# goldbricklemon/uplift-upsample-3dhpe

Hardware: AMD Instinct MI355X
Metric: pose-sequences/sec (higher is better)
Workload: dtype f16x3 (f32 operands split into f16 hi/lo, 3 MFMA passes, f32 accumulate); 1 GPU; config/h36m_351.json forward, N=71 tokens (receptive field 351), J=17, batch 128/GPU, s_in=5, seeded Keras-default weights; global_batch=128, parallelism=batch-sharded x1, hipgraph=True, concurrent_half_batches=False, batches_in_flight=8

## Files before the change

### uplift-upsample-3dhpe_amd/build.py

```python
import os
import subprocess
import sys

HERE = os.path.dirname(os.path.abspath(__file__))
CSRC = os.path.join(HERE, "csrc")
LIB = os.path.join(CSRC, "libuu3d.so")
SOURCES = ["uu3d_api.hip", "uu3d_ops.hip"]
HEADERS = ["uu3d_tchain16.h", "uu3d_gemm.h", "uu3d_gemm_h3.h", "uu3d_gemm_panel.h", "uu3d_gemm_panel8.h", "uu3d_gemm_wt.h", "uu3d_mlp_fused.h", "uu3d_attn.h", "uu3d_attn_h3.h", "uu3d_attn_long.h", "uu3d_spatial.h", "uu3d_spatial_h3.h", "uu3d_pk.h", "uu3d_misc.h", "uu3d_train.h", "uu3d_bwd.h", "uu3d_launch.h", "uu3d_train_kernels.h", "uu3d_dropout.h", "uu3d_train_step.inc", os.path.join("..", "..", "include", "uu3d_ops.h"), os.path.join("..", "..", "include", "uu3d.h")]


def _fingerprint(extra_flags=()):
    import hashlib
    h = hashlib.sha256()
    for f in SOURCES + HEADERS:
        h.update(f.encode()); h.update(open(os.path.join(CSRC, f), "rb").read())
    h.update(repr((DEVICE_FLAGS, tuple(extra_flags))).encode())
    try:
        h.update(subprocess.run([os.environ.get("HIPCC", "/opt/rocm/bin/hipcc"), "--version"], capture_output=True, text=True).stdout.encode())
    except OSError:
        pass
    return h.hexdigest()


def _stale(lib, extra_flags=()):
    stamp = lib + ".sha256"
    if not os.path.exists(lib) or not os.path.exists(stamp):
        return True
    return open(stamp).read().strip() != _fingerprint(extra_flags)


DEVICE_FLAGS = ["-Xclang", "-target-feature", "-Xclang", "-packed-fp32-ops"]
_HOST_NOISE = "is not a recognized feature for this target"


TIMING_LIB = os.path.join(CSRC, "libuu3d_timing.so")


def build(force=False, verbose=False, extra_flags=(), timing=False):
    lib = TIMING_LIB if timing else LIB
    extra_flags = tuple(extra_flags) + (("-DUU3D_TIMING_BUILD",) if timing else ())
    if not force and not _stale(lib, extra_flags):
        return lib
    hipcc = os.environ.get("HIPCC", "/opt/rocm/bin/hipcc")
    cmd = [hipcc, "-O3", "-std=c++17", "--offload-arch=gfx950", "-shared", "-fPIC",
           "-Wall", "-Wno-unused-function", *DEVICE_FLAGS, *extra_flags,
           "-o", lib] + [os.path.join(CSRC, s) for s in SOURCES]
    if verbose:
        print(" ".join(cmd), flush=True)
    r = subprocess.run(cmd, cwd=CSRC, stderr=subprocess.PIPE, text=True)
    err = "".join(l for l in r.stderr.splitlines(True) if _HOST_NOISE not in l)
    if err.strip():
        sys.stderr.write(err)
    if r.returncode != 0:
        raise subprocess.CalledProcessError(r.returncode, cmd)
    with open(lib + ".sha256", "w") as f:
        f.write(_fingerprint(extra_flags) + "\n")
    return lib


if __name__ == "__main__":
    print(build(force="--force" in sys.argv, verbose=True, timing="--timing" in sys.argv))
# ... 1 lines not shown
```

### uplift-upsample-3dhpe_amd/csrc/uu3d_api.hip

```cpp
#include <hip/hip_runtime.h>

#include <algorithm>
#include <cmath>
#include <cstdio>
#include <cstdlib>
#include <cstring>
#include <functional>
#include <map>
#include <string>
#include <vector>

#include "../../include/uu3d.h"
#include "uu3d_gemm.h"
#include "uu3d_gemm_h3.h"
#include "uu3d_gemm_panel.h"
#include <mutex>
#include "uu3d_gemm_panel8.h"
#include "uu3d_gemm_wt.h"
#include "uu3d_mlp_fused.h"
#include "uu3d_tchain16.h"
#include "uu3d_attn.h"
#include "uu3d_attn_h3.h"
#include "uu3d_spatial.h"
#include "uu3d_spatial_h3.h"
#include "uu3d_misc.h"
#include "uu3d_train.h"
#include "uu3d_bwd.h"
#include "uu3d_launch.h"
#include "uu3d_train_kernels.h"

using namespace uu3d;

namespace {

constexpr int kJ = 17, kDS = 32, kHS = 64, kHeads = 8, kDH = 48;
using SLY = SpatialBlockLayout<kDS, kHS>;
using SLY2 = SpatialBlockLayoutV2<kDS, kHS>;
constexpr int kFR = 3;
#ifndef UU3D_SPATIAL_MT
#define UU3D_SPATIAL_MT 1
#endif
constexpr int kSpatialMT = UU3D_SPATIAL_MT;

std::string g_create_error;

inline int round_up(int v, int m) { return (v + m - 1) / m * m; }
inline size_t align_up(size_t v, size_t a) { return (v + a - 1) / a * a; }

struct WeightRec {
    std::string name;
    std::vector<int64_t> dims;
    int64_t numel = 0;
    std::vector<float> host;
    bool set = false;
};

struct BlockDev {
    const float *ln1_g, *ln1_b, *wqkv_t, *bqkv, *wp_t, *bp, *ln2_g, *ln2_b, *w1_t, *b1, *w2_t, *b2;
    const float* pe;
    size_t wqkv_pf = 0, w1_pf = 0;
    size_t w2_mf = 0;
    size_t wp_pf = 0;
};

struct ProfRec {
    std::string name, kernel;
    double flops, bytes;
    hipEvent_t e0, e1;
};

}

struct uu3d_train_state;
struct uu3d_model {
    uu3d_config cfg;
    uu3d_train_state* ts = nullptr;
    int device = 0;
    std::vector<WeightRec> weights;
    std::map<std::string, int> index;
    std::vector<int> L;
    bool committed = false;
    bool generic = false;
    float* gparams = nullptr;
    float* arena = nullptr;
    size_t arena_floats = 0;
    bool no_mlpf = false;
    bool no_wt = false;
    bool attn_f32 = false;
    bool attn_wg = false;
    bool no_panel = false;
    bool no_panel_proj = false;
    bool throughput = false;
    struct TcLaunch { int flags; size_t w_off ; size_t p_off ; };
    std::vector<TcLaunch> tchain;
    int tchain_mode = -1;
    int tchain_min_tiles = 8;
    bool tchain_short = true;
    int num_cus = 256;
    std::recursive_mutex train_mu;
    bool in_commit = false;
    int* d_range = nullptr;
    bool no_planes = false;
    _Float16* harena = nullptr;
    size_t harena_halfs = 0;
    std::map<size_t, std::pair<size_t, size_t>> hplanes;
    std::map<size_t, size_t> panel_off, mlpf_off;
    SpatialParams sp{};
    const float* sp_blocks_v1 = nullptr;
    const float* sp_blocks_v2 = nullptr;
    bool spatial_valu = false;
    bool spatial_f32 = false;
    bool spatial_h3_always = false;
    size_t sp_frag_off = 0;
    const float *s2t_wt = nullptr, *s2t_b = nullptr, *token = nullptr, *pe_t = nullptr;
    std::vector<BlockDev> tblocks, sblocks;
    const float *h1_wt = nullptr, *h1_b = nullptr, *h2_wt = nullptr, *h2_b = nullptr;
    bool profiling = false;
    std::vector<ProfRec> prof;
    size_t prof_used = 0;
    std::string err;
};

namespace {

inline bool tchain_possible(const uu3d_config& c) {
    return c.precision == UU3D_PREC_F16X3 && c.d_temporal == 384 && c.h_temporal == 768 && c.num_heads == 8 && c.temporal_depth >= 1;
}

int fail(uu3d_model* m, int code, const std::string& msg) {
    if (m) m->err = msg; else g_create_error = msg;
    return code;
}

#define HIPCHK(m, expr)                                                                         \
    do {                                                                                        \
        hipError_t e__ = (expr);                                                                \
        if (e__ != hipSuccess)                                                                  \
            return fail(m, UU3D_ERR_HIP, std::string(#expr) + ": " + hipGetErrorString(e__));   \
    } while (0)

void add_weight(uu3d_model* m, const std::string& name, std::vector<int64_t> dims) {
    WeightRec r;
    r.name = name;
    r.dims = dims;
    r.numel = 1;
    for (auto d : dims) r.numel *= d;
    m->index[name] = (int)m->weights.size();
    m->weights.push_back(std::move(r));
}

void add_block(uu3d_model* m, const std::string& p, int d, int h, bool strided, bool qkv_bias) {
    add_weight(m, p + "/norm1/gamma", {d});
    add_weight(m, p + "/norm1/beta", {d});
    for (const char* nm : {"wq", "wk", "wv"}) {
        add_weight(m, p + "/attn/" + nm + "/kernel", {d, d});
        if (qkv_bias) add_weight(m, p + "/attn/" + nm + "/bias", {d});
    }
    add_weight(m, p + "/attn/projection/kernel", {d, d});
    add_weight(m, p + "/attn/projection/bias", {d});
    add_weight(m, p + "/norm2/gamma", {d});
    add_weight(m, p + "/norm2/beta", {d});
    if (strided) {
        add_weight(m, p + "/mlp/fc1/kernel", {1, d, h});
        add_weight(m, p + "/mlp/fc1/bias", {h});
        add_weight(m, p + "/mlp/strided_conv/kernel", {3, h, d});
        add_weight(m, p + "/mlp/strided_conv/bias", {d});
// ... 105 lines not shown
    if (generic) {
        if (c->num_heads < 1 || c->d_spatial < 1 || c->d_temporal < 1 || c->h_spatial < 1 || c->h_temporal < 1)
            return fail(nullptr, UU3D_ERR_INVALID_ARGUMENT, "dims and head count must be positive");
        if (c->d_spatial % c->num_heads != 0 || c->d_temporal % c->num_heads != 0)
            return fail(nullptr, UU3D_ERR_INVALID_ARGUMENT, "embed dims must be divisible by NUM_HEADS (vision_transformer.py:79)");
        if (!attn_generic_head_dim_ok(c->d_spatial / c->num_heads) || !attn_generic_head_dim_ok(c->d_temporal / c->num_heads))
            return fail(nullptr, UU3D_ERR_UNSUPPORTED, "generic forward: head dims (embed dim / NUM_HEADS) must be one of 2, 4, 8, 12, 16, 24, 32, 48, 64");
        if (c->d_spatial % 4 != 0 || c->d_temporal % 4 != 0 || c->h_spatial % 4 != 0)
            return fail(nullptr, UU3D_ERR_UNSUPPORTED, "generic forward: embed dims and MLP widths must be multiples of 4 (16-byte row pieces in every loader)");
        if (c->num_keypoints > 128 || c->num_frames > 128)
            return fail(nullptr, UU3D_ERR_UNSUPPORTED, "generic forward: at most 128 keypoints and 128 frames");
        if (c->temporal_depth < 1 || c->num_strided < 1 || !c->full_output)
            return fail(nullptr, UU3D_ERR_UNSUPPORTED, "generic forward: needs at least one temporal block, one strided block and the full-sequence head");
    }
    if (c->h_temporal % 4 != 0 || c->h_temporal < 4)
        return fail(nullptr, UU3D_ERR_UNSUPPORTED, "h_temporal must be a positive multiple of 4");
    if (c->temporal_depth == 0 && c->has_strided_input && c->num_strided > 0 && c->first_strided_token_attention_layer > 1)
        return fail(nullptr, UU3D_ERR_INVALID_ARGUMENT, "temporal_depth == 0 with FIRST_STRIDED_TOKEN_ATTENTION_LAYER > 1: the reference's key mask has N entries, strided block 2 has fewer keys");
    if (c->d_temporal > 64 * 4 * 4)
        return fail(nullptr, UU3D_ERR_UNSUPPORTED, "d_temporal > 1024");

    int ndev = 0;
    if (hipGetDeviceCount(&ndev) != hipSuccess || device < 0 || device >= ndev)
        return fail(nullptr, UU3D_ERR_NO_DEVICE, "HIP device not available");

    auto* m = new uu3d_model();
    m->cfg = *c;
    m->device = device;
    m->generic = generic;
    m->L.push_back(c->num_frames);
    for (int i = 0; i < c->num_strided; ++i) {
        if (c->strides[i] < 1 || c->pad_left[i] < 0 || c->pad_right[i] < 0) {
            delete m;
            return fail(nullptr, UU3D_ERR_INVALID_ARGUMENT, "bad stride/padding");
        }
        const int Lin = m->L.back();
        const int Lout = (Lin + c->pad_left[i] + c->pad_right[i] - 3) / c->strides[i] + 1;
        if (Lin + c->pad_left[i] + c->pad_right[i] < 3 || Lout < 1) {
            delete m;
            return fail(nullptr, UU3D_ERR_INVALID_ARGUMENT, "strided block reduces the sequence below one token");
        }
        if (Lin > (c->precision == UU3D_PREC_F16X3 ? ATTN_H3_MAX_L : 128)) {
            delete m;
            return fail(nullptr, UU3D_ERR_UNSUPPORTED, c->precision == UU3D_PREC_F16X3 ? "sequence length > 416 tokens" : "sequence length > 128 tokens with precision f32");
        }
        m->L.push_back(Lout);
    }
    if (c->num_strided > 0 && m->L.back() != 1) {
        delete m;
        return fail(nullptr, UU3D_ERR_INVALID_ARGUMENT, "STRIDES/PADDINGS must reduce the sequence to one token");
    }
    build_inventory(m);
    { const char* e = getenv("UU3D_SPATIAL"); m->spatial_valu = (e != nullptr && std::string(e) == "valu");
      m->spatial_f32 = (e != nullptr && std::string(e) == "f32"); m->spatial_h3_always = (e != nullptr && std::string(e) == "h3"); }
    { const char* e = getenv("UU3D_NO_PLANES"); m->no_planes = (e != nullptr && e[0] == '1'); }
    { const char* e = getenv("UU3D_ATTN_WG"); m->attn_wg = (e != nullptr && e[0] == '1'); }
    { const char* e = getenv("UU3D_NO_MLPF"); m->no_mlpf = (e != nullptr && e[0] == '1'); }
    { const char* e = getenv("UU3D_NO_WT"); m->no_wt = (e != nullptr && e[0] == '1'); }
    { const char* e = getenv("UU3D_ATTN_F32"); m->attn_f32 = (e != nullptr && e[0] == '1'); }
    { const char* e = getenv("UU3D_NO_PANEL"); m->no_panel = (e != nullptr && e[0] == '1'); }
    { const char* e = getenv("UU3D_NO_PANEL_PROJ"); m->no_panel_proj = (e != nullptr && e[0] == '1'); }
    { const char* e = getenv("UU3D_TCHAIN"); if (e != nullptr && (e[0] == '0' || e[0] == '1')) m->tchain_mode = e[0] - '0'; }
    { const char* e = getenv("UU3D_TCHAIN_MIN_TILES"); if (e != nullptr && atoi(e) > 0) m->tchain_min_tiles = atoi(e); }
    { const char* e = getenv("UU3D_TCHAIN_SHORT"); if (e != nullptr) m->tchain_short = atoi(e) != 0; }
    { hipDeviceProp_t pr; if (hipGetDeviceProperties(&pr, device) == hipSuccess && pr.multiProcessorCount > 0) m->num_cus = pr.multiProcessorCount; }
    if (hipSetDevice(device) != hipSuccess) {
        delete m;
        return fail(nullptr, UU3D_ERR_HIP, "hipSetDevice failed");
    }
    if (hipMalloc((void**)&m->d_range, 2 * sizeof(int)) != hipSuccess || hipMemset(m->d_range, 0, 2 * sizeof(int)) != hipSuccess) {
        delete m;
        return fail(nullptr, UU3D_ERR_HIP, "hipMalloc of the range-guard word failed");
    }
    *out = m;
    return UU3D_OK;
}

static void train_free(uu3d_model* m);
static int generic_forward(uu3d_model* m, const float* kp2d, const uint8_t* mask, int32_t B, float* full_out, float* central_out,
                           float* const* attn_out, void* workspace, size_t workspace_bytes, void* stream);
void uu3d_destroy(uu3d_model* m) {
    if (!m) return;
    (void)hipSetDevice(m->device);
    train_free(m);
    if (m->gparams) (void)hipFree(m->gparams);
    if (m->arena) (void)hipFree(m->arena);
    if (m->harena) (void)hipFree(m->harena);
    if (m->d_range) (void)hipFree(m->d_range);
    for (auto& r : m->prof) { (void)hipEventDestroy(r.e0); (void)hipEventDestroy(r.e1); }
    delete m;
}

int uu3d_num_weights(const uu3d_model* m) { return m ? (int)m->weights.size() : 0; }

int uu3d_weight_info(const uu3d_model* m, int i, const char** name, int32_t* ndim, int64_t dims[4]) {
    if (!m || i < 0 || i >= (int)m->weights.size()) return UU3D_ERR_INVALID_ARGUMENT;
    const WeightRec& r = m->weights[i];
    if (name) *name = r.name.c_str();
    if (ndim) *ndim = (int32_t)r.dims.size();
    if (dims) for (size_t k = 0; k < 4; ++k) dims[k] = k < r.dims.size() ? r.dims[k] : 1;
    return UU3D_OK;
}

int uu3d_set_weight(uu3d_model* m, const char* name, const float* data, int64_t numel) {
    if (!m || !name || !data) return fail(m, UU3D_ERR_INVALID_ARGUMENT, "null argument to uu3d_set_weight");
    auto it = m->index.find(name);
    if (it == m->index.end()) return fail(m, UU3D_ERR_INVALID_ARGUMENT, std::string("unknown weight: ") + name);
// ... 241 lines not shown
            add_proj(tb, block_name(true, 0)); add_fc1(tb, block_name(true, 0));
            tcb.push_back(std::move(tb));
        }
    }

    if (m->arena_floats < P.buf.size()) {
        if (m->arena) HIPCHK(m, hipFree(m->arena));
        m->arena = nullptr;
        HIPCHK(m, hipMalloc((void**)&m->arena, P.buf.size() * sizeof(float)));
        m->arena_floats = P.buf.size();
    }
    HIPCHK(m, hipMemcpyAsync(m->arena, P.buf.data(), P.buf.size() * sizeof(float), hipMemcpyHostToDevice, stream));
    HIPCHK(m, hipStreamSynchronize(stream));
    if (c.precision == UU3D_PREC_F16X3) {
        std::vector<_Float16> hb(64, (_Float16)0.f);
        m->hplanes.clear();
        for (auto& d : P.dense) {
            const size_t hi = align_up(hb.size(), 64); hb.resize(hi + d.second);
            const size_t lo = align_up(hb.size(), 64); hb.resize(lo + d.second);
            for (size_t i = 0; i < d.second; ++i) {
                const float x = P.buf[d.first + i];
                if (!(std::fabs(x) < 65504.0f))
                    return fail(m, UU3D_ERR_RANGE, "a Dense / Conv1D kernel holds a value of magnitude >= 65504 (or a non-finite one): not representable by the f16x3 operand planes; build the model with precision f32");
                const _Float16 h = h3_hi(x);
                hb[hi + i] = h; hb[lo + i] = (_Float16)((x - (float)h) * H3_SCALE);
            }
            m->hplanes[d.first] = {hi, lo};
        }
        {
            using FL = SpatialFragLayoutH3;
            m->sp_frag_off = align_up(hb.size(), 64);
            hb.resize(m->sp_frag_off + (size_t)c.spatial_depth * FL::size);
            for (int i = 0; i < c.spatial_depth; ++i) {
                const std::string p = "spatial_block_" + std::to_string(i + 1);
                _Float16* d = hb.data() + m->sp_frag_off + (size_t)i * FL::size;
                auto frag = [&](int off, const std::string& nm, int K, int Nn) {
                    const float* s = W(m, p + nm);
                    for (int nt = 0; nt < Nn / 32; ++nt)
                        for (int kk = 0; kk < K / 16; ++kk)
                            for (int lane = 0; lane < 64; ++lane)
                                for (int e = 0; e < 8; ++e) {
                                    const float x = s[(size_t)(16 * kk + 8 * (lane >> 5) + e) * Nn + 32 * nt + (lane & 31)];
                                    const _Float16 h = h3_hi(x);
                                    const size_t at = (size_t)off + (((size_t)(nt * (K / 16) + kk) * 2) * 64 + lane) * 8 + e;
                                    d[at] = h;
                                    d[at + 64 * 8] = (_Float16)((x - (float)h) * H3_SCALE);
                                }
                };
                frag(FL::fq, "/attn/wq/kernel", ds, ds); frag(FL::fk, "/attn/wk/kernel", ds, ds);
                frag(FL::fv, "/attn/wv/kernel", ds, ds); frag(FL::fp, "/attn/projection/kernel", ds, ds);
                frag(FL::f1, "/mlp/fc1/kernel", ds, kHS); frag(FL::f2, "/mlp/fc2/kernel", kHS, ds);
            }
        }
        m->panel_off.clear();
        if (dt % 192 == 0 && ht % 32 == 0) {
            auto add_panel = [&](size_t bt_off, int Nn, int K = 0, int Kp = 0) {
                if (K == 0) { K = dt; Kp = Kdt; }
                const auto it = m->hplanes.find(bt_off);
                if (it == m->hplanes.end() || K % 384 != 0) return;
                const size_t at = align_up(hb.size(), 64);
                hb.resize(at + panel_b_halfs(Nn, K));
                panel_pack_operand(hb.data() + it->second.first, hb.data() + it->second.second, Nn, K, Kp, hb.data() + at);
                m->panel_off[bt_off] = at;
            };
            for (auto& o : toff) { add_panel(o.wqkv, 3 * dt); add_panel(o.w1, ht); add_panel(o.wp, dt); }
            m->mlpf_off.clear();
            if (dt == 32 * MLPF_OC && ht == 256 * MLPF_SLICES)
                for (auto& o : toff) {
                    const auto it = m->hplanes.find(o.w2);
                    if (it == m->hplanes.end()) continue;
                    const size_t at = align_up(hb.size(), 64);
                    hb.resize(at + mlpf_w2_halfs());
                    mlpf_pack_w2(hb.data() + it->second.first, hb.data() + it->second.second, Kht, hb.data() + at);
                    m->mlpf_off[o.w2] = at;
                }
            for (auto& o : soff) { add_panel(o.wqkv, 3 * dt); add_panel(o.w1, ht); add_panel(o.wp, dt); }
        }
        m->tchain.clear();
        for (auto& tb : tcb) {
            const size_t at = align_up(hb.size(), 128);
            hb.resize(at + (size_t)tchain_chunks(tb.flags) * TC_CHUNK_HALFS);
            size_t o = at;
            for (auto& st : tb.stages) {
                std::vector<_Float16> Bh((size_t)st.N * st.K), Bl((size_t)st.N * st.K);
                const bool qkv_stage = st.N == 3 * dt;
                for (int n = 0; n < st.N; ++n)
                    for (int k = 0; k < st.K; ++k) {
                        const float x = st.Wk[(size_t)k * st.N + n] * (qkv_stage && n < dt ? tc_qscale : 1.0f);
                        if (!(std::fabs(x) < 65504.0f)) return fail(m, UU3D_ERR_RANGE, "a LayerNorm-folded kernel of the temporal chain leaves the f16 range; build the model with precision f32");
                        const _Float16 h = h3_hi(x);
                        Bh[(size_t)n * st.K + k] = h; Bl[(size_t)n * st.K + k] = (_Float16)((x - (float)h) * H3_SCALE);
                    }
                tchain16_pack_stage(Bh.data(), Bl.data(), st.N, st.K, st.kofs, st.natural, hb.data() + o);
                o += (size_t)(st.N / 32) * TC_CHUNK_HALFS;
            }
            if (tb.flags & TC_MLP) {
                _Float16* mlp = hb.data() + at + (size_t)((tb.flags & TC_PROJ) ? 12 : 0) * TC_CHUNK_HALFS;
                const std::vector<_Float16> tmp(mlp, mlp + (size_t)48 * TC_CHUNK_HALFS);
                tchain16_reorder_mlp(tmp.data(), mlp);
            }
            m->tchain.push_back({tb.flags, at, tb.p_off});
        }
        if (m->harena_halfs < hb.size()) {
            if (m->harena) HIPCHK(m, hipFree(m->harena));
            m->harena = nullptr;
            HIPCHK(m, hipMalloc((void**)&m->harena, hb.size() * sizeof(_Float16)));
// ... 512 lines not shown
        return fail(m, UU3D_ERR_INVALID_ARGUMENT, "stride_mask must be given iff the model has strided input");
    const bool has_h1 = c.full_output && c.temporal_depth > 0;
    if (has_h1 && !full_out) return fail(m, UU3D_ERR_INVALID_ARGUMENT, "full_out_dev is required for this model");
    if (((uintptr_t)workspace & 255) != 0) return fail(m, UU3D_ERR_WORKSPACE, "workspace must be 256-byte aligned");
    if (m->generic) {
        const int r = generic_forward(m, kp2d, mask, B, full_out, central_out, attn_out, workspace, workspace_bytes, stream_);
        if (r == UU3D_OK && c.precision == UU3D_PREC_F16X3) {
            const bool has_full = c.full_output && c.temporal_depth > 0 && full_out != nullptr;
            hipLaunchKernelGGL(range_check_kernel, dim3(256), dim3(256), 0, (hipStream_t)stream_, has_full ? full_out : central_out,
                               has_full ? (long)B * c.num_frames * c.num_keypoints * 3 : 0L, central_out, (long)B * c.num_keypoints * 3, m->d_range);
        }
        return r;
    }
    Workspace w = carve(m, B, (char*)workspace);
    if (workspace_bytes < w.bytes) return fail(m, UU3D_ERR_WORKSPACE, "workspace smaller than uu3d_workspace_bytes(batch)");
    if ((long)B * c.num_frames * c.num_keypoints > (1L << 30)) return fail(m, UU3D_ERR_INVALID_ARGUMENT, "batch too large");

    HIPCHK(m, hipSetDevice(m->device));
    Launcher Lh{m, (hipStream_t)stream_, w.slab, w.slab_floats, schedule == UU3D_SCHEDULE_THROUGHPUT, c.precision};
    m->prof_used = 0;
    const int N = c.num_frames, J = c.num_keypoints, ds = c.d_spatial, dt = c.d_temporal, ht = c.h_temporal;
    const int M = B * N;
    char nm[48];

    if (frames != nullptr && !part_tail) {
        Lh.begin("frames_to_tokens", "frames_to_tokens", 0.0, 4.0 * 3.0 * M * dt);
        hipLaunchKernelGGL(frames_to_tokens_kernel, dim3((unsigned)(((size_t)M * (dt / 4) + 255) / 256)), dim3(256), 0, Lh.stream,
                           frames->features, frames->num_rows, frames->rows, mask, m->token, m->pe_t, (long)M, N, dt, w.X);
        Lh.end();
    }
    const bool s2t_planes = !m->no_planes && c.precision == UU3D_PREC_F16X3 && !m->spatial_valu && !m->spatial_f32 && (m->spatial_h3_always || spatial_h3_pays(B * c.num_frames)) && ((c.num_keypoints * c.d_spatial) % 32 == 0);
    if (frames == nullptr && !part_tail) {
        SpatialParams sp = m->sp;
        sp.total_frames = M;
        sp.frame_list = nullptr;
        if (mask != nullptr && !m->spatial_valu) {
            Lh.begin("compact_frames", "compact_frames", 0.0, (double)M * 5.0);
            hipLaunchKernelGGL(compact_frames_kernel, dim3(1), dim3(1024), 0, Lh.stream, mask, M, w.frame_list);
            Lh.end();
            sp.frame_list = w.frame_list;
        }
        const double fl = (double)M * (2.0 * J * 2 * ds + c.spatial_depth * (4.0 * 2 * J * ds * ds + 8.0 * 4 * J * J * (ds / 8) + 2.0 * 2 * J * ds * kHS));
        if (m->spatial_valu) {
            constexpr int FPW = 256 / kJ;
            sp.blocks = m->sp_blocks_v1;
            auto kern = spatial_stack_kernel<kJ, kDS, kHS, kHeads>;
            static bool attr_done = false;
            if (!attr_done) { (void)hipFuncSetAttribute((const void*)kern, hipFuncAttributeMaxDynamicSharedMemorySize, (int)spatial_lds_bytes(kDS)); attr_done = true; }
            Lh.begin("spatial_stack", "spatial_valu", fl, 4.0 * M * J * (2.0 + ds));
            hipLaunchKernelGGL(kern, dim3((M + FPW - 1) / FPW), dim3(256), spatial_lds_bytes(kDS), Lh.stream, kp2d, sp, w.S);
            Lh.end();
        } else if (c.precision == UU3D_PREC_F16X3 && !m->spatial_f32 && (m->spatial_h3_always || spatial_h3_pays(M))) {
            sp.blocks = m->sp_blocks_v2;
            auto kern = spatial_stack_h3_kernel<kJ, kFR, kSpatialMT>;
            Lh.begin("spatial_stack", "spatial_h3", fl, 4.0 * M * J * (2.0 + ds));
            if (!(skip_mask() & 1))
            hipLaunchKernelGGL(kern, dim3((M + kFR - 1) / kFR), dim3(64 * (2 / kSpatialMT)), sh3::lds_bytes(), Lh.stream, kp2d, sp,
                               m->harena + m->sp_frag_off, w.S, s2t_planes ? reinterpret_cast<_Float16*>(w.S) : (_Float16*)nullptr,
                               s2t_planes ? reinterpret_cast<_Float16*>(w.S) + (size_t)M * J * ds : (_Float16*)nullptr, SpatialTrainIO{});
            Lh.end();
        } else {
            sp.blocks = m->sp_blocks_v2;
            auto kern = spatial_stack_mfma_kernel<kJ, kFR>;
            Lh.begin("spatial_stack", "spatial_mfma", fl, 4.0 * M * J * (2.0 + ds));
            hipLaunchKernelGGL(kern, dim3((M + kFR - 1) / kFR), dim3(64), spatial_v2_lds_bytes(), Lh.stream, kp2d, sp, w.S);
            Lh.end();
        }
    }
    if (frames == nullptr && !part_tail) {
        EpSpatialToTemporal ep{w.X, m->s2t_b, dt, mask, m->token, m->pe_t, N};
        if (s2t_planes) {
            Lh.gemm_g("s2t", GLoadPlain{reinterpret_cast<const _Float16*>(w.S), reinterpret_cast<const _Float16*>(w.S) + (size_t)M * J * ds, J * ds, M}, m->s2t_wt, M, dt, J * ds, ep);
        } else {
            ALoadPlain al{w.S, J * ds, M, J * ds};
            Lh.gemm("s2t", al, m->s2t_wt, M, dt, J * ds, ep);
        }
    }
    const bool planes = (c.precision == UU3D_PREC_F16X3) && (dt % 32 == 0) && (ht % 32 == 0) && !m->no_planes;
    constexpr int kFewRows = 512;
    _Float16* const Ph = reinterpret_cast<_Float16*>(w.O);
    _Float16* const Hh = reinterpret_cast<_Float16*>(w.Hb);
    const _Float16* const hzero = m->harena;

    auto block_head = [&](const char* tag, int i, const BlockDev& b, float* x, int L, const uint8_t* kmask, const BlockDev* pend, bool fuse_mlp) -> const _Float16* {
        const int Mr = B * L;
        auto name = [&](const char* what) { snprintf(nm, sizeof nm, "%s%d.%s", tag, i + 1, what); return nm; };
        _Float16* const Pl = Ph + (size_t)Mr * dt; _Float16* const Hl = Hh + (size_t)Mr * ht;
        const bool qsplit = Lh.attn_is_h3(L, planes);
        _Float16* const Qh = reinterpret_cast<_Float16*>(w.QKV); _Float16* const Ql = Qh + (size_t)Mr * 3 * dt;
        const EpBiasSplitQ ep_qs{Qh, Ql, b.bqkv, 3 * dt, dt, Lh.attn_qscale()};
        const bool few = planes && Mr <= kFewRows && Lh.wt_ok(b.wqkv_t, dt) && Lh.wt_ok(b.w1_t, dt);
        auto maps = [&]() {
            if (attn_out != nullptr && tag[0] == 't' && attn_out[i] != nullptr) {
                Lh.begin(name("attn_maps"), "attn_probs", 2.0 * B * (double)c.num_heads * L * L * kDH, 4.0 * B * (double)c.num_heads * L * L);
                const size_t lds = (size_t)L * (kDH + 1) * sizeof(float);
                static const bool once = (hipFuncSetAttribute((const void*)attn_probs_kernel, hipFuncAttributeMaxDynamicSharedMemorySize, 160 * 1024 - 256) == hipSuccess); (void)once;
                if (qsplit) hipLaunchKernelGGL(attn_probs_kernel, dim3(B * c.num_heads), dim3(256), lds, Lh.stream, (const void*)Qh, (const _Float16*)Ql, 3 * dt, dt, L, c.num_heads, kDH, kmask, 1.0f, 1, attn_out[i]);
                else hipLaunchKernelGGL(attn_probs_kernel, dim3(B * c.num_heads), dim3(256), lds, Lh.stream, (const void*)w.QKV, (const _Float16*)nullptr, 3 * dt, dt, L, c.num_heads, kDH, kmask, 1.0f / sqrtf((float)kDH), 0, attn_out[i]);
                Lh.end();
            }
        };
        if (few) {
            WtLoadF32 l1{x, dt, Mr, dt, b.ln1_g, b.ln1_b, 1e-5f, 1};
            if (qsplit) Lh.gemm_wt(name("ln_qkv"), l1, b.wqkv_t, Mr, 3 * dt, dt, ep_qs);
            else Lh.gemm_wt(name("ln_qkv"), l1, b.wqkv_t, Mr, 3 * dt, dt, EpBias{w.QKV, b.bqkv, 3 * dt});
            maps();
            Lh.attn(name("attn"), w.QKV, B, L, kmask, w.O, (size_t)Mr * dt);
            { GLoadPlain gl{Ph, Pl, dt, Mr}; Lh.gemm_g(name("proj_res"), gl, b.wp_t, Mr, dt, dt, EpBiasResidual{x, b.bp, dt, nullptr, nullptr, 1}, 4.0 * Mr * dt); }
            WtLoadF32 l2{x, dt, Mr, dt, b.ln2_g, b.ln2_b, 1e-5f, 1};
            Lh.gemm_wt(name("ln_fc1"), l2, b.w1_t, Mr, ht, dt, EpBiasReluSplit{Hh, Hl, b.b1, ht});
            return nullptr;
        }
        if (pend != nullptr) {
// ... 146 lines not shown
    auto take = [&](size_t n) { size_t o = off; off = align_up(off + n, 256); return o; };
    FrameWorkspace w{};
    const size_t oS = take((size_t)F * c.num_keypoints * c.d_spatial * 4);
    w.slab_floats = (size_t)1536 * 4096;
    const size_t oSl = take(w.slab_floats * 4);
    w.bytes = off;
    if (base) { w.S = (float*)(base + oS); w.slab = (float*)(base + oSl); }
    return w;
}
}

size_t uu3d_frame_features_bytes(const uu3d_model* m, int32_t frames) {
    if (!m || frames < 1 || m->generic) return 0;
    return carve_frames(m, frames, nullptr).bytes;
}

int uu3d_frame_features(uu3d_model* m, const float* frames_dev, int32_t F, float* features, void* workspace, size_t workspace_bytes,
                        int32_t schedule, void* stream_) {
    if (!m) return UU3D_ERR_INVALID_ARGUMENT;
    const bool exact_f32 = (schedule & UU3D_SCHEDULE_EXACT_F32) != 0;
    schedule &= ~UU3D_SCHEDULE_EXACT_F32;
    if (schedule != UU3D_SCHEDULE_LATENCY && schedule != UU3D_SCHEDULE_THROUGHPUT) return fail(m, UU3D_ERR_INVALID_ARGUMENT, "schedule must be UU3D_SCHEDULE_LATENCY or UU3D_SCHEDULE_THROUGHPUT");
    if (m->generic) return fail(m, UU3D_ERR_UNSUPPORTED, "uu3d_frame_features: handles with generic dims have no frames form (compiled dims only)");
    if (!m->committed) return fail(m, UU3D_ERR_NOT_READY, "uu3d_commit_weights has not been called");
    if (!frames_dev || !features || !workspace || F < 1) return fail(m, UU3D_ERR_INVALID_ARGUMENT, "null buffer or frames < 1");
    if ((long)F * m->cfg.num_keypoints > (1L << 30)) return fail(m, UU3D_ERR_INVALID_ARGUMENT, "too many frames");
    if (((uintptr_t)workspace & 255) != 0) return fail(m, UU3D_ERR_WORKSPACE, "workspace must be 256-byte aligned");
    const FrameWorkspace w = carve_frames(m, F, (char*)workspace);
    if (workspace_bytes < w.bytes) return fail(m, UU3D_ERR_WORKSPACE, "workspace smaller than uu3d_frame_features_bytes(frames)");
    uu3d_config c = m->cfg;
    if (exact_f32) c.precision = UU3D_PREC_F32;
    HIPCHK(m, hipSetDevice(m->device));
    Launcher Lh{m, (hipStream_t)stream_, w.slab, w.slab_floats, schedule == UU3D_SCHEDULE_THROUGHPUT, c.precision};
    m->prof_used = 0;
    const int J = c.num_keypoints, ds = c.d_spatial, dt = c.d_temporal;
    const int M = F;
    const bool h3 = c.precision == UU3D_PREC_F16X3 && !m->spatial_valu && !m->spatial_f32 && (m->spatial_h3_always || spatial_h3_pays(M));
    const bool s2t_planes = h3 && !m->no_planes && ((J * ds) % 32 == 0);
    SpatialParams sp = m->sp;
    sp.total_frames = M;
    sp.frame_list = nullptr;
    const double fl = (double)M * (2.0 * J * 2 * ds + c.spatial_depth * (4.0 * 2 * J * ds * ds + 8.0 * 4 * J * J * (ds / 8) + 2.0 * 2 * J * ds * kHS));
    if (m->spatial_valu) {
        constexpr int FPW = 256 / kJ;
        sp.blocks = m->sp_blocks_v1;
        auto kern = spatial_stack_kernel<kJ, kDS, kHS, kHeads>;
        static bool attr_done = false;
        if (!attr_done) { (void)hipFuncSetAttribute((const void*)kern, hipFuncAttributeMaxDynamicSharedMemorySize, (int)spatial_lds_bytes(kDS)); attr_done = true; }
        Lh.begin("spatial_stack", "spatial_valu", fl, 4.0 * M * J * (2.0 + ds));
        hipLaunchKernelGGL(kern, dim3((M + FPW - 1) / FPW), dim3(256), spatial_lds_bytes(kDS), Lh.stream, frames_dev, sp, w.S);
        Lh.end();
    } else if (h3) {
        sp.blocks = m->sp_blocks_v2;
        auto kern = spatial_stack_h3_kernel<kJ, kFR, kSpatialMT>;
        Lh.begin("spatial_stack", "spatial_h3", fl, 4.0 * M * J * (2.0 + ds));
        hipLaunchKernelGGL(kern, dim3((M + kFR - 1) / kFR), dim3(64 * (2 / kSpatialMT)), sh3::lds_bytes(), Lh.stream, frames_dev, sp,
                           m->harena + m->sp_frag_off, w.S, s2t_planes ? reinterpret_cast<_Float16*>(w.S) : (_Float16*)nullptr,
                           s2t_planes ? reinterpret_cast<_Float16*>(w.S) + (size_t)M * J * ds : (_Float16*)nullptr, SpatialTrainIO{});
        Lh.end();
    } else {
        sp.blocks = m->sp_blocks_v2;
        auto kern = spatial_stack_mfma_kernel<kJ, kFR>;
        Lh.begin("spatial_stack", "spatial_mfma", fl, 4.0 * M * J * (2.0 + ds));
        hipLaunchKernelGGL(kern, dim3((M + kFR - 1) / kFR), dim3(64), spatial_v2_lds_bytes(), Lh.stream, frames_dev, sp, w.S);
        Lh.end();
    }
    const EpBias ep{features, m->s2t_b, dt};
    if (s2t_planes) Lh.gemm_g("s2t", GLoadPlain{reinterpret_cast<const _Float16*>(w.S), reinterpret_cast<const _Float16*>(w.S) + (size_t)M * J * ds, J * ds, M}, m->s2t_wt, M, dt, J * ds, ep);
    else { ALoadPlain al{w.S, J * ds, M, J * ds}; Lh.gemm("s2t", al, m->s2t_wt, M, dt, J * ds, ep); }
    if (c.precision == UU3D_PREC_F16X3) {
        Lh.begin("range_check", "range_check", 0.0, 4.0 * (double)M * dt);
        hipLaunchKernelGGL(range_check_kernel, dim3(256), dim3(256), 0, Lh.stream, features, (long)M * dt, features, 0L, m->d_range);
        Lh.end();
    }
    return Lh.status;
}

int uu3d_range_status(uu3d_model* m, void* stream, int32_t* out_flag) {
    if (!m) return UU3D_ERR_INVALID_ARGUMENT;
    HIPCHK(m, hipSetDevice(m->device));
    int h = 0;
    hipLaunchKernelGGL(range_take_kernel, dim3(1), dim3(1), 0, (hipStream_t)stream, m->d_range, m->d_range + 1);
    HIPCHK(m, hipMemcpyAsync(&h, m->d_range + 1, sizeof(int), hipMemcpyDeviceToHost, (hipStream_t)stream));
    HIPCHK(m, hipStreamSynchronize((hipStream_t)stream));
    if (out_flag) *out_flag = h != 0;
    if (h != 0) return fail(m, UU3D_ERR_RANGE, "non-finite values in a forward's outputs: activations beyond the f16 range (65504) of the f16x3 products, or non-finite inputs "
                                               "(repeat the batch with UU3D_SCHEDULE_EXACT_F32 or build the model with precision f32)");
    return UU3D_OK;
}

int uu3d_mpjpe(const float* pred, const float* gt, int32_t B, int32_t J, int32_t root, double* out, void* stream) {
    if (!pred || !gt || !out || B < 1 || J < 1 || root < 0 || root >= J) return UU3D_ERR_INVALID_ARGUMENT;
    hipLaunchKernelGGL(mpjpe_kernel, dim3((B * J + 255) / 256), dim3(256), 0, (hipStream_t)stream, pred, gt, B, J, root, out);
    return hipGetLastError() == hipSuccess ? UU3D_OK : UU3D_ERR_HIP;
}

int uu3d_gather_windows(const float* poses, const int64_t* video_start, const int32_t* video_len, const uu3d_window* windows,
                        const int32_t* flip_order, int32_t B, int32_t N, int32_t J, int32_t Cc, int32_t pad_edge,
                        int32_t zero_masked, float* out, uint8_t* stride_mask, uint8_t* pad_mask, void* stream) {
    if (!poses || !video_start || !video_len || !windows || !out || !stride_mask || B < 1 || N < 1 || J < 1 || Cc < 1 || Cc > 4)
        return UU3D_ERR_INVALID_ARGUMENT;
    static_assert(sizeof(uu3d_window) == sizeof(WindowDesc), "descriptor layouts must agree");
    const long total = (long)B * N * J;
    hipLaunchKernelGGL(gather_windows_kernel, dim3((unsigned)((total + 255) / 256)), dim3(256), 0, (hipStream_t)stream,
                       poses, video_start, video_len, reinterpret_cast<const WindowDesc*>(windows), flip_order,
                       B, N, J, Cc, pad_edge, zero_masked, out, stride_mask, pad_mask);
    return hipGetLastError() == hipSuccess ? UU3D_OK : UU3D_ERR_HIP;
}

int uu3d_gather_window_frames(const int64_t* video_start, const int32_t* video_len, const uu3d_window* windows, int32_t B, int32_t N,
                              int32_t pad_edge, int32_t zero_masked, int64_t frame_base, int64_t zero_row, int32_t* rows,
                              uint8_t* stride_mask, uint8_t* pad_mask, void* stream) {
// ... 98 lines not shown
```

Baseline: 208,100 pose-sequences/s.

## Add per-token 16x16x32 MFMA spatial stack kernel with pre-split f16 weight fragments

```diff
diff --git a/uplift-upsample-3dhpe_amd/build.py b/uplift-upsample-3dhpe_amd/build.py
--- a/uplift-upsample-3dhpe_amd/build.py
+++ b/uplift-upsample-3dhpe_amd/build.py
@@ -6,7 +6,7 @@
 CSRC = os.path.join(HERE, "csrc")
 LIB = os.path.join(CSRC, "libuu3d.so")
 SOURCES = ["uu3d_api.hip", "uu3d_ops.hip"]
-HEADERS = ["uu3d_tchain16.h", "uu3d_gemm.h", "uu3d_gemm_h3.h", "uu3d_gemm_panel.h", "uu3d_gemm_panel8.h", "uu3d_gemm_wt.h", "uu3d_mlp_fused.h", "uu3d_attn.h", "uu3d_attn_h3.h", "uu3d_attn_long.h", "uu3d_spatial.h", "uu3d_spatial_h3.h", "uu3d_pk.h", "uu3d_misc.h", "uu3d_train.h", "uu3d_bwd.h", "uu3d_launch.h", "uu3d_train_kernels.h", "uu3d_dropout.h", "uu3d_train_step.inc", os.path.join("..", "..", "include", "uu3d_ops.h"), os.path.join("..", "..", "include", "uu3d.h")]
+HEADERS = ["uu3d_tchain16.h", "uu3d_gemm.h", "uu3d_gemm_h3.h", "uu3d_gemm_panel.h", "uu3d_gemm_panel8.h", "uu3d_gemm_wt.h", "uu3d_mlp_fused.h", "uu3d_attn.h", "uu3d_attn_h3.h", "uu3d_attn_long.h", "uu3d_spatial.h", "uu3d_spatial_h3.h", "uu3d_spatial_p16.h", "uu3d_pk.h", "uu3d_misc.h", "uu3d_train.h", "uu3d_bwd.h", "uu3d_launch.h", "uu3d_train_kernels.h", "uu3d_dropout.h", "uu3d_train_step.inc", os.path.join("..", "..", "include", "uu3d_ops.h"), os.path.join("..", "..", "include", "uu3d.h")]
 
 
 def _fingerprint(extra_flags=()):
diff --git a/uplift-upsample-3dhpe_amd/csrc/uu3d_api.hip b/uplift-upsample-3dhpe_amd/csrc/uu3d_api.hip
--- a/uplift-upsample-3dhpe_amd/csrc/uu3d_api.hip
+++ b/uplift-upsample-3dhpe_amd/csrc/uu3d_api.hip
@@ -23,6 +23,7 @@
 #include "uu3d_attn_h3.h"
 #include "uu3d_spatial.h"
 #include "uu3d_spatial_h3.h"
+#include "uu3d_spatial_p16.h"
 #include "uu3d_misc.h"
 #include "uu3d_train.h"
 #include "uu3d_bwd.h"
@@ -40,6 +41,7 @@
 #ifndef UU3D_SPATIAL_MT
 #define UU3D_SPATIAL_MT 1
 #endif
+constexpr int kP16FR = 7, kP16PW = 1;
 constexpr int kSpatialMT = UU3D_SPATIAL_MT;
 
 std::string g_create_error;
@@ -112,6 +114,8 @@
     bool spatial_f32 = false;
     bool spatial_h3_always = false;
     size_t sp_frag_off = 0;
+    size_t sp_frag16_off = 0;
+    bool spatial_h3_tiles = false;
     const float *s2t_wt = nullptr, *s2t_b = nullptr, *token = nullptr, *pe_t = nullptr;
     std::vector<BlockDev> tblocks, sblocks;
     const float *h1_wt = nullptr, *h1_b = nullptr, *h2_wt = nullptr, *h2_b = nullptr;
@@ -323,7 +327,8 @@
     }
     build_inventory(m);
     { const char* e = getenv("UU3D_SPATIAL"); m->spatial_valu = (e != nullptr && std::string(e) == "valu");
-      m->spatial_f32 = (e != nullptr && std::string(e) == "f32"); m->spatial_h3_always = (e != nullptr && std::string(e) == "h3"); }
+      m->spatial_f32 = (e != nullptr && std::string(e) == "f32"); m->spatial_h3_always = (e != nullptr && std::string(e) == "h3");
+      m->spatial_h3_tiles = (e != nullptr && std::string(e) == "h3tiles"); }
     { const char* e = getenv("UU3D_NO_PLANES"); m->no_planes = (e != nullptr && e[0] == '1'); }
     { const char* e = getenv("UU3D_ATTN_WG"); m->attn_wg = (e != nullptr && e[0] == '1'); }
     { const char* e = getenv("UU3D_NO_MLPF"); m->no_mlpf = (e != nullptr && e[0] == '1'); }
@@ -671,6 +676,31 @@
                 frag(FL::f1, "/mlp/fc1/kernel", ds, kHS); frag(FL::f2, "/mlp/fc2/kernel", kHS, ds);
             }
         }
+        {
+            using FL = SpatialFragLayoutP16;
+            m->sp_frag16_off = align_up(hb.size(), 64);
+            hb.resize(m->sp_frag16_off + (size_t)c.spatial_depth * FL::size);
+            for (int i = 0; i < c.spatial_depth; ++i) {
+                const std::string p = "spatial_block_" + std::to_string(i + 1);
+                _Float16* d = hb.data() + m->sp_frag16_off + (size_t)i * FL::size;
+                auto frag = [&](int off, const std::string& nm, int K, int Nn) {
+                    const float* s = W(m, p + nm);
+                    for (int nt = 0; nt < Nn / 16; ++nt)
+                        for (int ks = 0; ks < K / 32; ++ks)
+                            for (int lane = 0; lane < 64; ++lane)
+                                for (int j = 0; j < 8; ++j) {
+                                    const float x = s[(size_t)p16_kch(ks, lane >> 4, j) * Nn + 16 * nt + (lane & 15)];
+                                    const _Float16 h = h3_hi(x);
+                                    const size_t at = (size_t)off + (((size_t)(nt * (K / 32) + ks) * 2) * 64 + lane) * 8 + j;
+                                    d[at] = h;
+                                    d[at + 64 * 8] = (_Float16)((x - (float)h) * H3_SCALE);
+                                }
+                };
+                frag(FL::fq, "/attn/wq/kernel", ds, ds); frag(FL::fk, "/attn/wk/kernel", ds, ds);
+                frag(FL::fv, "/attn/wv/kernel", ds, ds); frag(FL::fp, "/attn/projection/kernel", ds, ds);
+                frag(FL::f1, "/mlp/fc1/kernel", ds, kHS); frag(FL::f2, "/mlp/fc2/kernel", kHS, ds);
+            }
+        }
         m->panel_off.clear();
         if (dt % 192 == 0 && ht % 32 == 0) {
             auto add_panel = [&](size_t bt_off, int Nn, int K = 0, int Kp = 0) {
@@ -1289,13 +1319,23 @@
             Lh.end();
         } else if (c.precision == UU3D_PREC_F16X3 && !m->spatial_f32 && (m->spatial_h3_always || spatial_h3_pays(M))) {
             sp.blocks = m->sp_blocks_v2;
-            auto kern = spatial_stack_h3_kernel<kJ, kFR, kSpatialMT>;
-            Lh.begin("spatial_stack", "spatial_h3", fl, 4.0 * M * J * (2.0 + ds));
-            if (!(skip_mask() & 1))
-            hipLaunchKernelGGL(kern, dim3((M + kFR - 1) / kFR), dim3(64 * (2 / kSpatialMT)), sh3::lds_bytes(), Lh.stream, kp2d, sp,
-                               m->harena + m->sp_frag_off, w.S, s2t_planes ? reinterpret_cast<_Float16*>(w.S) : (_Float16*)nullptr,
-                               s2t_planes ? reinterpret_cast<_Float16*>(w.S) + (size_t)M * J * ds : (_Float16*)nullptr, SpatialTrainIO{});
-            Lh.end();
+            _Float16* s_hi = s2t_planes ? reinterpret_cast<_Float16*>(w.S) : (_Float16*)nullptr;
+            _Float16* s_lo = s2t_planes ? reinterpret_cast<_Float16*>(w.S) + (size_t)M * J * ds : (_Float16*)nullptr;
+            if (m->spatial_h3_tiles) {
+                auto kern = spatial_stack_h3_kernel<kJ, kFR, kSpatialMT>;
+                Lh.begin("spatial_stack", "spatial_h3", fl, 4.0 * M * J * (2.0 + ds));
+                if (!(skip_mask() & 1))
+                hipLaunchKernelGGL(kern, dim3((M + kFR - 1) / kFR), dim3(64 * (2 / kSpatialMT)), sh3::lds_bytes(), Lh.stream, kp2d, sp,
+                                   m->harena + m->sp_frag_off, w.S, s_hi, s_lo, SpatialTrainIO{});
+                Lh.end();
+            } else {
+                auto kern = spatial_stack_p16_kernel<kJ, kP16FR, kP16PW>;
+                Lh.begin("spatial_stack", "spatial_p16", fl, 4.0 * M * J * (2.0 + ds));
+                if (!(skip_mask() & 1))
+                hipLaunchKernelGGL(kern, dim3((M + kP16FR - 1) / kP16FR), dim3(64 * p16_waves(kJ, kP16FR, kP16PW)), sp16::lds_bytes<kP16FR>(c.spatial_depth),
+                                   Lh.stream, kp2d, sp, m->harena + m->sp_frag16_off, w.S, s_hi, s_lo);
+                Lh.end();
+            }
         } else {
             sp.blocks = m->sp_blocks_v2;
             auto kern = spatial_stack_mfma_kernel<kJ, kFR>;
@@ -1548,12 +1588,21 @@
         Lh.end();
     } else if (h3) {
         sp.blocks = m->sp_blocks_v2;
-        auto kern = spatial_stack_h3_kernel<kJ, kFR, kSpatialMT>;
-        Lh.begin("spatial_stack", "spatial_h3", fl, 4.0 * M * J * (2.0 + ds));
-        hipLaunchKernelGGL(kern, dim3((M + kFR - 1) / kFR), dim3(64 * (2 / kSpatialMT)), sh3::lds_bytes(), Lh.stream, frames_dev, sp,
-                           m->harena + m->sp_frag_off, w.S, s2t_planes ? reinterpret_cast<_Float16*>(w.S) : (_Float16*)nullptr,
-                           s2t_planes ? reinterpret_cast<_Float16*>(w.S) + (size_t)M * J * ds : (_Float16*)nullptr, SpatialTrainIO{});
-        Lh.end();
+        _Float16* s_hi = s2t_planes ? reinterpret_cast<_Float16*>(w.S) : (_Float16*)nullptr;
+        _Float16* s_lo = s2t_planes ? reinterpret_cast<_Float16*>(w.S) + (size_t)M * J * ds : (_Float16*)nullptr;
+        if (m->spatial_h3_tiles) {
+            auto kern = spatial_stack_h3_kernel<kJ, kFR, kSpatialMT>;
+            Lh.begin("spatial_stack", "spatial_h3", fl, 4.0 * M * J * (2.0 + ds));
+            hipLaunchKernelGGL(kern, dim3((M + kFR - 1) / kFR), dim3(64 * (2 / kSpatialMT)), sh3::lds_bytes(), Lh.stream, frames_dev, sp,
+                               m->harena + m->sp_frag_off, w.S, s_hi, s_lo, SpatialTrainIO{});
+            Lh.end();
+        } else {
+            auto kern = spatial_stack_p16_kernel<kJ, kP16FR, kP16PW>;
+            Lh.begin("spatial_stack", "spatial_p16", fl, 4.0 * M * J * (2.0 + ds));
+            hipLaunchKernelGGL(kern, dim3((M + kP16FR - 1) / kP16FR), dim3(64 * p16_waves(kJ, kP16FR, kP16PW)), sp16::lds_bytes<kP16FR>(c.spatial_depth),
+                               Lh.stream, frames_dev, sp, m->harena + m->sp_frag16_off, w.S, s_hi, s_lo);
+            Lh.end();
+        }
     } else {
         sp.blocks = m->sp_blocks_v2;
         auto kern = spatial_stack_mfma_kernel<kJ, kFR>;
diff --git a/uplift-upsample-3dhpe_amd/csrc/uu3d_spatial_p16.h b/uplift-upsample-3dhpe_amd/csrc/uu3d_spatial_p16.h
--- /dev/null
+++ b/uplift-upsample-3dhpe_amd/csrc/uu3d_spatial_p16.h
@@ -0,0 +1,322 @@
+#pragma once
+#include "uu3d_spatial_h3.h"
+
+namespace uu3d {
+
+struct SpatialFragLayoutP16 {
+    static constexpr int frag = 64 * 8;
+    static constexpr int fq = 0, fk = fq + 2 * 1 * 2 * frag, fv = fk + 2 * 1 * 2 * frag, fp = fv + 2 * 1 * 2 * frag;
+    static constexpr int f1 = fp + 2 * 1 * 2 * frag;
+    static constexpr int f2 = f1 + 4 * 1 * 2 * frag;
+    static constexpr int size = f2 + 2 * 2 * 2 * frag;
+};
+__host__ __device__ inline constexpr int p16_kch(int s, int g, int j) { return 32 * s + 16 * (j >> 2) + 4 * g + (j & 3); }
+__host__ __device__ inline constexpr int p16_waves(int J, int FR, int PW) { return (J * FR + 16 * PW - 1) / (16 * PW); }
+
+namespace sp16 {
+constexpr int NPARAM = sh3::NPARAM;
+constexpr int KFLD = 9 * sh3::KPLD + sh3::KFPAD;
+template <int FR>
+__host__ __device__ inline constexpr size_t lds_bytes(int depth) { return (size_t)2 * FR * KFLD * 4 + (size_t)depth * NPARAM * 4; }
+
+template <int NT, int KS>
+struct WF { h16x8 h[NT][KS], l[NT][KS]; };
+template <int NT, int KS>
+__device__ __forceinline__ void load_w(const _Float16* __restrict__ wf, const int lane, WF<NT, KS>& w) {
+    const h16x8* base = reinterpret_cast<const h16x8*>(wf) + lane;
+#pragma unroll
+    for (int nt = 0; nt < NT; ++nt)
+#pragma unroll
+        for (int s = 0; s < KS; ++s) {
+            w.h[nt][s] = base[((nt * KS + s) * 2 + 0) * 64];
+            w.l[nt][s] = base[((nt * KS + s) * 2 + 1) * 64];
+        }
+}
+
+__device__ __forceinline__ void frag_of(const f32x2* v, h16x8& bh, h16x8& bl) {
+    h16x4 h0, l0, h1, l1;
+    sh3::split_pairs(v[0], v[1], h0, l0);
+    sh3::split_pairs(v[2], v[3], h1, l1);
+    bh = (h16x8){h0[0], h0[1], h0[2], h0[3], h1[0], h1[1], h1[2], h1[3]};
+    bl = (h16x8){l0[0], l0[1], l0[2], l0[3], l1[0], l1[1], l1[2], l1[3]};
+    asm volatile("s_nop 1" : "+v"(bh), "+v"(bl));
+}
+
+template <int PW, int NT, int KS>
+__device__ __forceinline__ void mm(const WF<NT, KS>& w, const h16x8 (&bh)[PW][KS], const h16x8 (&bl)[PW][KS], f32x2 (&out)[PW][2 * NT]) {
+    f32x4 acc0[PW][NT], acc1[PW][NT];
+#pragma unroll
+    for (int pp = 0; pp < PW; ++pp)
+#pragma unroll
+        for (int nt = 0; nt < NT; ++nt) { acc0[pp][nt] = (f32x4){0.f, 0.f, 0.f, 0.f}; acc1[pp][nt] = acc0[pp][nt]; }
+#pragma unroll
+    for (int s = 0; s < KS; ++s)
+#pragma unroll
+        for (int nt = 0; nt < NT; ++nt)
+#pragma unroll
+            for (int pp = 0; pp < PW; ++pp) {
+                acc0[pp][nt] = __builtin_amdgcn_mfma_f32_16x16x32_f16(w.h[nt][s], bh[pp][s], acc0[pp][nt], 0, 0, 0);
+                acc1[pp][nt] = __builtin_amdgcn_mfma_f32_16x16x32_f16(w.h[nt][s], bl[pp][s], acc1[pp][nt], 0, 0, 0);
+                acc1[pp][nt] = __builtin_amdgcn_mfma_f32_16x16x32_f16(w.l[nt][s], bh[pp][s], acc1[pp][nt], 0, 0, 0);
+            }
+#pragma unroll
+    for (int pp = 0; pp < PW; ++pp)
+#pragma unroll
+        for (int nt = 0; nt < NT; ++nt) pk::behind_fence(acc0[pp][nt], acc1[pp][nt]);
+    asm volatile("s_nop 15\n\ts_nop 3" ::: "memory");
+#pragma unroll
+    for (int pp = 0; pp < PW; ++pp)
+#pragma unroll
+        for (int nt = 0; nt < NT; ++nt) pk::behind_fence(acc0[pp][nt], acc1[pp][nt]);
+    const f32x2 inv = pk::splat(1.0f / H3_SCALE);
+#pragma unroll
+    for (int pp = 0; pp < PW; ++pp)
+#pragma unroll
+        for (int nt = 0; nt < NT; ++nt)
+#pragma unroll
+            for (int e = 0; e < 2; ++e)
+                out[pp][2 * nt + e] = pk::fma((f32x2){acc1[pp][nt][2 * e], acc1[pp][nt][2 * e + 1]}, inv,
+                                              (f32x2){acc0[pp][nt][2 * e], acc0[pp][nt][2 * e + 1]});
+}
+
+__device__ __forceinline__ float sum4(const f32x2 p) {
+    typedef unsigned u32x2 __attribute__((ext_vector_type(2)));
+    float v;
+    asm("v_add_f32 %0, %1, %2\n\ts_nop 1" : "=v"(v) : "v"(p[0]), "v"(p[1]));
+    const u32x2 r = __builtin_amdgcn_permlane16_swap(__float_as_uint(v), __float_as_uint(v), false, false);
+    const float h = __uint_as_float(r[0]) + __uint_as_float(r[1]);
+    const u32x2 s = __builtin_amdgcn_permlane32_swap(__float_as_uint(h), __float_as_uint(h), false, false);
+    return __uint_as_float(s[0]) + __uint_as_float(s[1]);
+}
+
+__device__ __forceinline__ void param_pairs(const float* b, const int g, f32x2* bp) {
+#pragma unroll
+    for (int u = 0; u < 2; ++u) {
+        const f32x4 b4 = *reinterpret_cast<const f32x4*>(b + 16 * u + 4 * g);
+        bp[2 * u] = (f32x2){b4[0], b4[1]}; bp[2 * u + 1] = (f32x2){b4[2], b4[3]};
+    }
+}
+
+__device__ __forceinline__ void ln_token(const f32x2 (&x)[4], const f32x2 (&gp)[4], const f32x2 (&bp)[4], const float eps, f32x2 (&y)[4]) {
+    const float mean = sum4(pk::add(pk::add(x[0], x[1]), pk::add(x[2], x[3]))) * (1.0f / 32.0f);
+    const f32x2 m2 = pk::splat(mean);
+    f32x2 q2;
+    { const f32x2 d = pk::sub(x[0], m2); q2 = pk::mul(d, d); }
+#pragma unroll
+    for (int i = 1; i < 4; ++i) { const f32x2 d = pk::sub(x[i], m2); q2 = pk::fma(d, d, q2); }
+    const float q = sum4(q2);
+    const float rstd = 1.0f / sqrtf(q * (1.0f / 32.0f) + eps);
+    const f32x2 r2 = pk::splat(rstd);
+#pragma unroll
+    for (int i = 0; i < 4; ++i) {
+        const f32x2 inv = pk::mul(r2, gp[i]);
+        y[i] = pk::fma(x[i], inv, pk::fnma(m2, inv, bp[i]));
+    }
+}
+}
+
+template <int J, int FR, int PW>
+__global__ void __launch_bounds__(64 * p16_waves(J, FR, PW)) UU3D_PK_TARGET
+spatial_stack_p16_kernel(const float* __restrict__ kp2d, const SpatialParams p, const _Float16* __restrict__ wfrag,
+                         float* __restrict__ out, _Float16* __restrict__ out_hi, _Float16* __restrict__ out_lo)
+{
+#pragma clang fp contract(off)
+    using namespace sp16;
+    h3_flush_f16_denormals();
+    constexpr int DS = 32, HS = 64, NP = (J + 1) / 2;
+    constexpr int NW = p16_waves(J, FR, PW);
+    static_assert(J == 17 && DS == 32 && HS == 64, "17 joints, d = 32, hidden 64");
+    using LY = SpatialBlockLayoutV2<DS, HS>;
+    using FL = SpatialFragLayoutP16;
+    extern __shared__ __attribute__((aligned(16))) unsigned char lds_raw[];
+    float* TK = reinterpret_cast<float*>(lds_raw);
+    float* TV = TK + FR * KFLD;
+    float* P = TV + FR * KFLD;
+
+    const int lane = threadIdx.x & 63, t = lane & 15, g = lane >> 4;
+    const int wave = __builtin_amdgcn_readfirstlane(threadIdx.x >> 6);
+    int nframes = p.total_frames;
+    if (p.frame_list != nullptr) {
+        nframes = p.frame_list[p.total_frames];
+        if ((int)blockIdx.x * FR >= nframes) return;
+    }
+    for (int k = threadIdx.x; k < p.depth * NPARAM; k += 64 * NW) P[k] = p.blocks[(size_t)(k / NPARAM) * LY::size + k % NPARAM];
+    for (int k = threadIdx.x; k < FR * 2 * DS; k += 64 * NW) {
+        const int f = k / (2 * DS), c = k % DS;
+        (k % (2 * DS) < DS ? TK : TV)[f * KFLD + (NP - 1) * sh3::KPLD + 2 * c + 1] = 0.f;
+    }
+    __syncthreads();
+
+    int frame[PW], joint[PW], kslot[PW];
+    unsigned kfr[PW];
+    bool valid[PW], real[PW];
+#pragma unroll
+    for (int pp = 0; pp < PW; ++pp) {
+        const int s = 16 * (PW * wave + pp) + t;
+        real[pp] = s < J * FR;
+        const int fl = real[pp] ? s / J : FR - 1;
+        joint[pp] = real[pp] ? s % J : J - 1;
+        int f = blockIdx.x * FR + fl;
+        valid[pp] = real[pp] && (f < nframes);
+        if (p.frame_list != nullptr) f = p.frame_list[min(f, nframes - 1)];
+        frame[pp] = min(f, p.total_frames - 1);
+        kslot[pp] = fl * KFLD + (joint[pp] >> 1) * sh3::KPLD + (joint[pp] & 1);
+        kfr[pp] = (unsigned)(fl * KFLD * 4);
+    }
+    const unsigned tk_a = (unsigned)(uintptr_t)(__attribute__((address_space(3))) const void*)TK;
+    const unsigned tv_a = (unsigned)(uintptr_t)(__attribute__((address_space(3))) const void*)TV;
+
+    f32x2 x[PW][4];
+#pragma unroll
+    for (int pp = 0; pp < PW; ++pp) {
+        float kx = 0.f, ky = 0.f;
+        if (valid[pp]) { const float2 k2 = *reinterpret_cast<const float2*>(kp2d + ((size_t)frame[pp] * J + joint[pp]) * 2); kx = k2.x; ky = k2.y; }
+        const f32x2 kx2 = pk::splat(kx), ky2 = pk::splat(ky);
+#pragma unroll
+        for (int i = 0; i < 4; ++i) {
+            const int c = 16 * (i >> 1) + 4 * g + 2 * (i & 1);
+            const f32x2 w0 = *reinterpret_cast<const f32x2*>(p.embed_w + c), w1 = *reinterpret_cast<const f32x2*>(p.embed_w + DS + c);
+            const f32x2 eb = *reinterpret_cast<const f32x2*>(p.embed_b + c), pe = *reinterpret_cast<const f32x2*>(p.pe + joint[pp] * DS + c);
+            x[pp][i] = pk::add(pk::add(pk::fma(ky2, w1, pk::mul(kx2, w0)), eb), pe);
+        }
+    }
+    auto wg_sync = [&]() __attribute__((always_inline)) {
+        asm volatile("s_waitcnt lgkmcnt(0)" ::: "memory");
+        __builtin_amdgcn_s_barrier();
+        asm volatile("" ::: "memory");
+    };
+    auto store_kv = [&](float* T, const f32x2 (&v)[PW][4]) __attribute__((always_inline)) {
+#pragma unroll
+        for (int pp = 0; pp < PW; ++pp) {
+            if (!real[pp]) continue;
+#pragma unroll
+            for (int i = 0; i < 4; ++i) {
+                const int c = 16 * (i >> 1) + 4 * g + 2 * (i & 1);
+                T[kslot[pp] + 2 * c] = v[pp][i][0]; T[kslot[pp] + 2 * c + 2] = v[pp][i][1];
+            }
+        }
+    };
+
+    for (int blk = 0; blk < p.depth; ++blk) {
+        const _Float16* __restrict__ F = wfrag + (size_t)blk * FL::size;
+        const float* W = P + blk * NPARAM;
+        WF<2, 1> wq, wk, wv, wp;
+        load_w(F + FL::fq, lane, wq); load_w(F + FL::fk, lane, wk); load_w(F + FL::fv, lane, wv);
+        f32x2 gp[4], bp[4];
+
+        h16x8 bh[PW][1], bl[PW][1];
+        param_pairs(W + LY::ln1_g, g, gp); param_pairs(W + LY::ln1_b, g, bp);
+#pragma unroll
+        for (int pp = 0; pp < PW; ++pp) {
+            f32x2 y[4];
+            ln_token(x[pp], gp, bp, 1e-5f, y);
+            frag_of(y, bh[pp][0], bl[pp][0]);
+        }
+        f32x2 q[PW][4];
+        {
+            f32x2 kv[PW][4];
+            mm<PW, 2, 1>(wq, bh, bl, q);
+            param_pairs(W + LY::bq, g, bp);
+#pragma unroll
+            for (int pp = 0; pp < PW; ++pp)
+#pragma unroll
+                for (int i = 0; i < 4; ++i) q[pp][i] = pk::add(q[pp][i], bp[i]);
+            mm<PW, 2, 1>(wk, bh, bl, kv);
+            param_pairs(W + LY::bk, g, bp);
+#pragma unroll
+            for (int pp = 0; pp < PW; ++pp)
+#pragma unroll
+                for (int i = 0; i < 4; ++i) kv[pp][i] = pk::add(kv[pp][i], bp[i]);
+            wg_sync();
+            store_kv(TK, kv);
+            load_w(F + FL::fp, lane, wp);
+            mm<PW, 2, 1>(wv, bh, bl, kv);
+            param_pairs(W + LY::bv, g, bp);
+#pragma unroll
+            for (int pp = 0; pp < PW; ++pp)
+#pragma unroll
+                for (int i = 0; i < 4; ++i) kv[pp][i] = pk::add(kv[pp][i], bp[i]);
+            store_kv(TV, kv);
+        }
+        wg_sync();
+        f32x2 o[PW][4];
+#pragma unroll
+        for (int pp = 0; pp < PW; ++pp)
+#pragma unroll
+            for (int u = 0; u < 2; ++u) {
+                const unsigned off = kfr[pp] + (unsigned)((16 * u + 4 * g) * 2 * 4);
+                f32x2 qa[1] = {q[pp][2 * u]}, qb[1] = {q[pp][2 * u + 1]}, oa[1], ob[1];
+                sh3::head_attention<J, 1>(qa, qb, tk_a + off, tv_a + off, oa, ob);
+                o[pp][2 * u] = oa[0]; o[pp][2 * u + 1] = ob[0];
+            }
+#pragma unroll
+        for (int pp = 0; pp < PW; ++pp) frag_of(o[pp], bh[pp][0], bl[pp][0]);
+        {
+            f32x2 pr[PW][4];
+            mm<PW, 2, 1>(wp, bh, bl, pr);
+            param_pairs(W + LY::bp, g, bp);
+#pragma unroll
+            for (int pp = 0; pp < PW; ++pp)
+#pragma unroll
+                for (int i = 0; i < 4; ++i) x[pp][i] = pk::add(x[pp][i], pk::add(pr[pp][i], bp[i]));
+        }
+
+        WF<4, 1> w1;
+        WF<2, 2> w2;
+        load_w(F + FL::f1, lane, w1);
+        load_w(F + FL::f2, lane, w2);
+        param_pairs(W + LY::ln2_g, g, gp); param_pairs(W + LY::ln2_b, g, bp);
+#pragma unroll
+        for (int pp = 0; pp < PW; ++pp) {
+            f32x2 y[4];
+            ln_token(x[pp], gp, bp, 1e-5f, y);
+            frag_of(y, bh[pp][0], bl[pp][0]);
+        }
+        h16x8 hh[PW][2], hl[PW][2];
+        {
+            f32x2 hd[PW][8], b1[8];
+            mm<PW, 4, 1>(w1, bh, bl, hd);
+            param_pairs(W + LY::b1, g, b1); param_pairs(W + LY::b1 + 32, g, b1 + 4);
+#pragma unroll
+            for (int pp = 0; pp < PW; ++pp) {
+#pragma unroll
+                for (int i = 0; i < 8; ++i) hd[pp][i] = sh3::gelu_pair(pk::add(hd[pp][i], b1[i]));
+#pragma unroll
+                for (int s = 0; s < 2; ++s) frag_of(hd[pp] + 4 * s, hh[pp][s], hl[pp][s]);
+            }
+        }
+        {
+            f32x2 z[PW][4];
+            mm<PW, 2, 2>(w2, hh, hl, z);
+            param_pairs(W + LY::b2, g, bp);
+#pragma unroll
+            for (int pp = 0; pp < PW; ++pp)
+#pragma unroll
+                for (int i = 0; i < 4; ++i) x[pp][i] = pk::add(x[pp][i], pk::add(z[pp][i], bp[i]));
+        }
+    }
+
+    f32x2 gp[4], bp[4];
+    param_pairs(p.norm_g, g, gp); param_pairs(p.norm_b, g, bp);
+#pragma unroll
+    for (int pp = 0; pp < PW; ++pp) {
+        f32x2 y[4];
+        ln_token(x[pp], gp, bp, 1e-6f, y);
+        if (!valid[pp]) continue;
+        const size_t at = ((size_t)frame[pp] * J + joint[pp]) * DS;
+#pragma unroll
+        for (int u = 0; u < 2; ++u) {
+            const int c = 16 * u + 4 * g;
+            if (out_lo != nullptr) {
+                h16x4 hi, lo;
+                sh3::split_pairs(y[2 * u], y[2 * u + 1], hi, lo);
+                *reinterpret_cast<h16x4*>(out_hi + at + c) = hi;
+                *reinterpret_cast<h16x4*>(out_lo + at + c) = lo;
+            } else {
+                *reinterpret_cast<f32x4*>(out + at + c) = (f32x4){y[2 * u][0], y[2 * u][1], y[2 * u + 1][0], y[2 * u + 1][1]};
+            }
+        }
+    }
+}
+
+}
```

Measured after the change: 217,500 pose-sequences/s (median of 6 runs). 1.05x the previous value.
